# ameli/gaussian-process-param-estimation

Hardware: AMD Instinct MI355X
Metric: log-likelihood evals/sec (N=16384 dense Matern-3/2) (higher is better)
Workload: dtype f64

## Files before the change

gaussian-process-param-estimation_amd/csrc/gpmi_api.hip:

```cpp

#include <hip/hip_runtime.h>

#include <algorithm>
#include <cmath>
#include <cstdarg>
#include <cstdio>
#include <cstdlib>
#include <cstring>
#include <array>
#include <map>
#include <vector>

#include "gpmi_internal.h"
#include "gpmi_host.h"
#include "gpmi_band.h"
#include "gpmi_dense_plan.h"
#include "gpmi_predict_plan.h"
#include "../../include/gpmi.h"

using namespace gpmi;

namespace {

thread_local char g_err[512] = "";

int set_err(int code, const char* fmt, ...) {
  va_list ap;
  va_start(ap, fmt);
  vsnprintf(g_err, sizeof(g_err), fmt, ap);
  va_end(ap);
  return code;
}

constexpr int TS = GPMI_TS;
constexpr int RLD = GPMI_RHS_LD;
constexpr int OUT_LD = 1 + RLD * RLD;

}

struct gpmi_op {
  int device = 0;
  int64_t n = 0, n_pad = 0;
  int nt = 0;
  int max_batch = 1;
  int outer = 16;
  int panel_mode = DENSE_REC;
  hipStream_t stream = nullptr;
  hipStream_t stream3 = nullptr;
  int groups = 0;
  hipEvent_t ev_g = nullptr;
  hipEvent_t ev_fork = nullptr, ev_join = nullptr;
  bool dry = false;
  std::vector<std::pair<int, int>> shapes;
  double* K = nullptr;
  double* A = nullptr;
  double* R = nullptr;
  double* X = nullptr;
  double* U = nullptr;
  double* Linv = nullptr;
  double* logdiag = nullptr;
  double* gram = nullptr;
  double* out = nullptr;
  double* etas = nullptr;
  double* rhs_src = nullptr;
  double* scratch = nullptr;
  double* scratch2 = nullptr;
  double* tracebuf = nullptr;
  double* W = nullptr;
  double* tpart = nullptr;
  double* Td = nullptr;
  int* info = nullptr;
  uint32_t* order = nullptr;
  int order_nt = -1, order_outer = -1, group = 8;
  std::map<std::pair<int, int>, int64_t> order_off;
  int nrhs = 0;
  bool has_K = false;
  bool cache_valid = false;
  double cached_eta = 0.0;
  uint64_t factor_gen = 0;
  uint64_t tinv_gen = ~0ull;
  int tinv_have = 0;
  double tinv[2] = {0.0, 0.0};
  double* PY = nullptr;
  double* PT = nullptr;
  double* Ppart = nullptr;
  double* Pout = nullptr;
  double* Pgram = nullptr;
  int pred_wide = 0;
  int64_t pred_t_rows = 0;
  double* Pcov = nullptr;
  double* Pcpart = nullptr;
  int64_t pred_cov_rows = 0;
  size_t pred_cpart = 0;
  int ncu = 0;
  hipEvent_t cov_ev[2] = {nullptr, nullptr};
  double last_cov_ms = 0.0, last_cov_flops = 0.0;
  int last_cov_split = 0;
  uint64_t rhs_gen = 0;
  uint64_t ry_gen = ~0ull;
  uint64_t ry_rhs = ~0ull;
  uint64_t py_gen = ~0ull, py_rhs = ~0ull;
  std::vector<hipEvent_t> pred_ev;
  double last_pred_ms = 0.0, last_pred_trail_ms = 0.0, last_pred_trail_flops = 0.0;
  bool timing = false;
  std::vector<hipEvent_t> ev;
  hipEvent_t ev_begin = nullptr, ev_end = nullptr;
  double last_syrk_ms = 0.0, last_syrk_flops = 0.0, last_total_ms = 0.0;
  int last_syrk_launches = 0;
  std::vector<std::pair<int, double>> syrk_log;
  std::vector<std::array<int, 3>> syrk_shape;
  double last_syrk_busy_ms = 0.0;
  bool trace = false;
  std::vector<hipEvent_t> colpanel_ev;
  size_t colpanel_ev_used = 0;

  BatchPtrs ptrs() const {
    BatchPtrs p;
    p.A = A;
    p.sA = n_pad * n_pad;
    p.R = R;
    p.sR = n_pad * RLD;
    p.U = U;
    p.sU = (int64_t)TS * RLD;
    p.Linv = Linv;
    p.sL = (int64_t)nt * TS * TS;
    p.logdiag = logdiag;
    p.sLD = nt;
    p.gram = gram;
    p.sG = (int64_t)nt * 256;
    p.info = info;
    return p;
  }
};

namespace {

void grouped_order(int w, int t, int G, std::vector<uint32_t>* out) {
  for (int r0 = 0; r0 < t; r0 += G) {
    const int r1 = std::min(t, r0 + G);
    const int jmax = std::min(r1 - 1, w - 1);
    for (int j = 0; j <= jmax; ++j)
      for (int i = std::max(r0, j); i < r1; ++i) out->push_back(((uint32_t)i << 16) | j);
  }
}

int launch_syrk(gpmi_op* op, hipStream_t st, int b0, int nb, int tc0, int w, int t, int p0,
                int kdim, bool from_k = false) {
  const int tri = w * (w + 1) / 2;
  const int tiles = tri + (t - w) * w;
  if (tiles <= 0 || nb <= 0) return 0;
  if (op->dry) {
    op->shapes.push_back({w, t});
    return 0;
  }
  int evi = -1;
  if (op->timing) {
    evi = (int)op->syrk_log.size() * 2;
    if ((int)op->ev.size() < evi + 2) {
      for (int k = 0; k < 64; ++k) {
        hipEvent_t e;
        HIP_TRY(hipEventCreateWithFlags(&e, timing_event_flags()));
        op->ev.push_back(e);
      }
    }
    HIP_TRY(hipEventRecord(op->ev[evi], st));
  }
  const uint32_t* order = nullptr;
  if (op->order && w > 1) {
    auto it = op->order_off.find({w, t});
    if (it != op->order_off.end()) order = op->order + it->second;
  }
  hipLaunchKernelGGL(syrk_kernel, dim3(tiles, nb), dim3(256), 0, st,
                     op->A + (int64_t)b0 * op->n_pad * op->n_pad, (int64_t)op->n_pad,
                     op->n_pad * op->n_pad, tc0, w, t, p0, kdim, order,
                     from_k ? op->K : nullptr, op->etas + b0, (int64_t)op->n);
  LAUNCH_CHECK("syrk_kernel");
  if (op->timing) {
    HIP_TRY(hipEventRecord(op->ev[evi + 1], st));
    const double offd = (double)(tiles - std::min(tiles, w)) * TS * TS;
    const double diag = (double)std::min(tiles, w) * TS * (TS + 1) / 2.0;
    const double fl = 2.0 * (offd + diag) * kdim * nb;
    op->syrk_log.push_back({evi, fl});
    op->syrk_shape.push_back({w, t, kdim});
  }
  return 0;
}

int factor_panel(gpmi_op* op, const BatchPtrs& P, int nb, hipStream_t st,
                 const DenseLaunch& L) {
  if (op->dry) return 0;
  const int64_t lda = op->n_pad;
  if (L.kind == DENSE_DIAG) {
    hipLaunchKernelGGL(diag_block_kernel, dim3(nb), dim3(256), 0, st, P, lda, L.col, op->nt);
    LAUNCH_CHECK("diag_block_kernel");
  } else if (L.kind == DENSE_PANEL) {
    hipLaunchKernelGGL(panel_kernel, dim3(L.r1 - L.r0, nb), dim3(256), 0, st, P, lda, L.col);
    LAUNCH_CHECK("panel_kernel");
  } else {
    const bool ev = op->timing && op->trace;
    size_t evi = op->colpanel_ev_used;
    if (ev) {
      while (op->colpanel_ev.size() < evi + 2) {
        hipEvent_t e;
        HIP_TRY(hipEventCreateWithFlags(&e, timing_event_flags()));
        op->colpanel_ev.push_back(e);
      }
      HIP_TRY(hipEventRecord(op->colpanel_ev[evi], st));
    }
    hipLaunchKernelGGL(colpanel_kernel, dim3(L.r1 - L.r0, nb), dim3(256), 0, st, P, lda, L.col,
                       L.p0 / TS, L.next_diag ? 1 : 0);
    LAUNCH_CHECK("colpanel_kernel");
    if (ev) {
      HIP_TRY(hipEventRecord(op->colpanel_ev[evi + 1], st));
      op->colpanel_ev_used = evi + 2;
    }
  }
  return 0;
}


int schedule(gpmi_op* op, const BatchPtrs& P, int b0, int nb, hipStream_t main = nullptr) {
  hipStream_t A = main ? main : op->stream;
  for (const DenseLaunch& L : dense_plan(op->nt, op->outer, op->panel_mode)) {
    const int rc = L.kind == DENSE_SYRK
                       ? launch_syrk(op, A, b0, nb, L.col, L.w, L.r1 - L.r0, L.p0, L.kdim,
                                     L.from_k)
                       : factor_panel(op, P, nb, A, L);
    if (rc) return rc;
  }
  return 0;
}

int ensure_order(gpmi_op* op) {
  if (op->group <= 0) return 0;
  if (op->order && op->order_nt == op->nt && op->order_outer == op->outer &&
      true)
    return 0;
  if (op->order) HIP_TRY(hipFree(op->order));
  op->order = nullptr;
  op->order_off.clear();
  op->dry = true;
  op->shapes.clear();
  BatchPtrs P = op->ptrs();
  int rc = schedule(op, P, 0, 1);
  op->dry = false;
  if (rc) return rc;
  std::vector<uint32_t> h;
  for (auto& wt : op->shapes) {
    if (wt.first < 2 || op->order_off.count(wt)) continue;
    op->order_off[wt] = (int64_t)h.size();
    grouped_order(wt.first, wt.second, op->group, &h);
  }
  if (h.empty()) h.push_back(0);
  HIP_TRY(hipMalloc(&op->order, sizeof(uint32_t) * h.size()));
  HIP_TRY(hipMemcpy(op->order, h.data(), sizeof(uint32_t) * h.size(), hipMemcpyHostToDevice));
// ... 225 lines not shown
  int rc = matern_params(nu, &P);
  if (rc) return rc;
  DeviceGuard g(device);
  double *dx = nullptr, *dv = nullptr;
  HIP_TRY(hipMalloc(&dx, sizeof(double) * m));
  HIP_TRY(hipMalloc(&dv, sizeof(double) * m));
  HIP_TRY(hipMemcpy(dx, x, sizeof(double) * m, hipMemcpyHostToDevice));
  hipLaunchKernelGGL(matern_eval_kernel, dim3((unsigned)((m + 255) / 256)), dim3(256), 0, 0, dx,
                     m, P, dv);
  LAUNCH_CHECK("matern_eval_kernel");
  HIP_TRY(hipMemcpy(out, dv, sizeof(double) * m, hipMemcpyDeviceToHost));
  HIP_TRY(hipFree(dx));
  HIP_TRY(hipFree(dv));
  return 0;
}

static int assemble(int device, hipStream_t s, const double* points, int64_t n, int d,
                    const double* scale, double nu, double* Kdev, int64_t ldk,
                    int64_t n_pad) {
  if (d < 1 || d > GPMI_MAX_DIM)
    return set_err(-1003, "dimension %d outside [1, %d]", d, GPMI_MAX_DIM);
  MaternParams P;
  int rc = matern_params(nu, &P);
  if (rc) return rc;
  DeviceGuard g(device);
  double *dp = nullptr, *ds = nullptr;
  HIP_TRY(hipMalloc(&dp, sizeof(double) * std::max<int64_t>(1, n * d)));
  HIP_TRY(hipMalloc(&ds, sizeof(double) * d));
  HIP_TRY(hipMemcpyAsync(dp, points, sizeof(double) * n * d, hipMemcpyHostToDevice, s));
  HIP_TRY(hipMemcpyAsync(ds, scale, sizeof(double) * d, hipMemcpyHostToDevice, s));
  const int64_t T = (n_pad + 63) / 64;
  hipEvent_t e0 = nullptr, e1 = nullptr;
  HIP_TRY(hipEventCreate(&e0));
  HIP_TRY(hipEventCreate(&e1));
  HIP_TRY(hipEventRecord(e0, s));
  launch_matern_dense(dim3((unsigned)(T * (T + 1) / 2)), s, dp, n, d, ds, P, Kdev, ldk, n_pad);
  LAUNCH_CHECK("matern_dense_kernel");
  HIP_TRY(hipEventRecord(e1, s));
  HIP_TRY(hipStreamSynchronize(s));
  float ms = 0.f;
  HIP_TRY(hipEventElapsedTime(&ms, e0, e1));
  g_assembly_ms = ms;
  HIP_TRY(hipEventDestroy(e0));
  HIP_TRY(hipEventDestroy(e1));
  HIP_TRY(hipFree(dp));
  HIP_TRY(hipFree(ds));
  return 0;
}

int gpmi_matern_dense(int device, const double* points, int64_t n, int d,
                      const double* scale, double nu, double* K_out, int64_t ldk) {
  if (n <= 0) return 0;
  DeviceGuard g(device);
  double* dK = nullptr;
  HIP_TRY(hipMalloc(&dK, sizeof(double) * n * n));
  int rc = assemble(device, nullptr, points, n, d, scale, nu, dK, n, n);
  if (rc) {
    (void)hipFree(dK);
    return rc;
  }
  HIP_TRY(hipMemcpy2D(K_out, sizeof(double) * ldk, dK, sizeof(double) * n, sizeof(double) * n,
                      n, hipMemcpyDeviceToHost));
  HIP_TRY(hipFree(dK));
  return 0;
}

int gpmi_op_create(int device, int64_t n, int max_batch, gpmi_op** out) {
  if (!out) return set_err(-1004, "null output handle");
  if (n <= 0) return set_err(-1005, "matrix size must be positive");
  if (max_batch < 1) max_batch = 1;
  DeviceGuard g(device);
  gpmi_op* op = new gpmi_op();
  op->device = device;
  op->n = n;
  op->n_pad = (n + TS - 1) / TS * TS;
  op->nt = (int)(op->n_pad / TS);
  op->max_batch = max_batch;
  if (const char* g = std::getenv("GPMI_GROUPS")) op->groups = std::atoi(g);
  if (const char* m = std::getenv("GPMI_PANEL")) {
    if (!std::strcmp(m, "col")) op->panel_mode = DENSE_COL;
    else if (std::strcmp(m, "rec") && *m) {
      delete op;
      return set_err(-1011, "GPMI_PANEL must be rec or col (got %s)", m);
    }
  }
  op->trace = std::getenv("GPMI_SYRK_TRACE") != nullptr;
  const int64_t np = op->n_pad;
  auto fail = [&](hipError_t e, const char* what) {
    gpmi_op_destroy(op);
    return set_err(-(int)e, "allocation of %s failed: %s", what, hipGetErrorString(e));
  };
  hipError_t e;
  if ((e = hipStreamCreateWithFlags(&op->stream, hipStreamNonBlocking)) != hipSuccess)
    return fail(e, "stream");
  if ((e = hipEventCreateWithFlags(&op->ev_fork, sync_event_flags())) != hipSuccess)
    return fail(e, "event");
  if ((e = hipEventCreateWithFlags(&op->ev_join, sync_event_flags())) != hipSuccess)
    return fail(e, "event");
#define ALLOC(ptr, count)                                                           \
  if ((e = hipMalloc(&op->ptr, sizeof(*op->ptr) * (size_t)(count))) != hipSuccess)  \
    return fail(e, #ptr);
  ALLOC(K, np * np);
  ALLOC(A, (size_t)max_batch * np * np);
  ALLOC(R, (size_t)max_batch * np * RLD);
  ALLOC(X, (size_t)max_batch * np * RLD);
  ALLOC(U, (size_t)max_batch * TS * RLD);
  ALLOC(Linv, (size_t)max_batch * op->nt * TS * TS);
  ALLOC(logdiag, (size_t)max_batch * op->nt);
  ALLOC(gram, (size_t)max_batch * op->nt * 256);
  ALLOC(out, (size_t)max_batch * OUT_LD);
  ALLOC(etas, max_batch);
  ALLOC(rhs_src, np * RLD);
  ALLOC(scratch, np * RLD);
  ALLOC(scratch2, np * RLD);
  ALLOC(tracebuf, np * 2);
  ALLOC(info, max_batch);
#undef ALLOC
  if ((e = hipMemsetAsync(op->rhs_src, 0, sizeof(double) * np * RLD, op->stream)) != hipSuccess)
    return fail(e, "rhs memset");
  if ((e = hipStreamSynchronize(op->stream)) != hipSuccess) return fail(e, "sync");
  *out = op;
  return 0;
}

int gpmi_op_destroy(gpmi_op* op) {
  if (!op) return 0;
  DeviceGuard g(op->device);
  if (op->stream) (void)hipStreamSynchronize(op->stream);
  if (op->stream3) (void)hipStreamSynchronize(op->stream3);
  double* bufs[] = {op->K, op->A, op->R, op->X, op->U, op->Linv, op->logdiag, op->gram,
                    op->out, op->etas, op->rhs_src, op->scratch, op->scratch2, op->tracebuf,
                    op->W, op->tpart, op->Td, op->PY, op->PT, op->Ppart, op->Pout, op->Pgram,
                    op->Pcov, op->Pcpart};
  for (double* p : bufs)
    if (p) (void)hipFree(p);
  if (op->info) (void)hipFree(op->info);
  if (op->order) (void)hipFree(op->order);
  for (auto e : op->ev) (void)hipEventDestroy(e);
  for (auto e : op->colpanel_ev) (void)hipEventDestroy(e);
  for (auto e : op->pred_ev) (void)hipEventDestroy(e);
  for (auto e : op->cov_ev)
    if (e) (void)hipEventDestroy(e);
  if (op->ev_begin) (void)hipEventDestroy(op->ev_begin);
  if (op->ev_end) (void)hipEventDestroy(op->ev_end);
  if (op->ev_fork) (void)hipEventDestroy(op->ev_fork);
  if (op->ev_join) (void)hipEventDestroy(op->ev_join);
  if (op->stream3) (void)hipStreamDestroy(op->stream3);
  if (op->ev_g) (void)hipEventDestroy(op->ev_g);
  if (op->stream) (void)hipStreamDestroy(op->stream);
  delete op;
  return 0;
}

int gpmi_op_size(const gpmi_op* op, int64_t* n, int64_t* n_pad) {
  if (!op) return set_err(-1006, "null handle");
  if (n) *n = op->n;
  if (n_pad) *n_pad = op->n_pad;
  return 0;
}

int gpmi_op_load_matrix(gpmi_op* op, const double* K_host, int64_t ldk) {
  if (!op) return set_err(-1006, "null handle");
  DeviceGuard g(op->device);
  const int64_t np = op->n_pad, n = op->n;
  std::vector<double> pad_rows;
  HIP_TRY(hipMemsetAsync(op->K, 0, sizeof(double) * np * np, op->stream));
// ... 671 lines not shown
```

gaussian-process-param-estimation_amd/csrc/gpmi_chol.hip:

```cpp

#include <hip/hip_runtime.h>
#include <math.h>
#include <stdint.h>

#include "gpmi_internal.h"

#include "gpmi_device.h"

namespace gpmi {

__global__ __launch_bounds__(256) void shift_copy_kernel(
    const double* __restrict__ K, int64_t ldk, double* __restrict__ A, int64_t lda,
    int64_t sA, const double* __restrict__ etas, int nb, int64_t n, int wc) {
  int I, J;
  tri_decode(blockIdx.x, wc, &I, &J);
  const int t = threadIdx.x;
  for (int e = t; e < TS * TS / 2; e += 256) {
    const int r = e >> 6, c = (e & 63) * 2;
    const int64_t gi = (int64_t)I * TS + r, gj = (int64_t)J * TS + c;
    const d2 v = *reinterpret_cast<const d2*>(K + gi * ldk + gj);
    for (int b = 0; b < nb; ++b) {
      d2 o = v;
      if (gi < n) {
        if (gi == gj) o[0] += etas[b];
// ... 48 lines not shown
#pragma unroll
  for (int it = 0; it < 4; ++it) v[it] = *reinterpret_cast<const d2*>(U + 2 * (it * 256 + t));
#pragma unroll
  for (int it = 0; it < 4; ++it) *reinterpret_cast<d2*>(&sU[2 * (it * 256 + t)]) = v[it];
}

__device__ __forceinline__ void wg_global_barrier() {
  __builtin_amdgcn_fence(__ATOMIC_RELEASE, "workgroup");
  __syncthreads();
  __builtin_amdgcn_fence(__ATOMIC_ACQUIRE, "workgroup");
}

__global__ __launch_bounds__(256, 2) void panel_kernel(BatchPtrs P, int64_t lda, int kb) {
  __shared__ double smem[4 * STAGE + TS * RLD];
  double* sU = smem + 4 * STAGE;
  const int b = blockIdx.y;
  const int I = kb + 1 + blockIdx.x;
  double* A = P.A + b * P.sA;
  if (!GPMI_PROBE_PANEL_NO_RHS) stage_u(P.U + b * P.sU, sU);
  panel_step(A + (int64_t)I * TS * lda + (int64_t)kb * TS, lda,
             P.Linv + b * P.sL + (int64_t)kb * TS * TS,
             P.R + b * P.sR + (int64_t)I * TS * RLD, smem, smem + 2 * STAGE, sU);
}

__device__ __forceinline__ void load_c(const double* C, int64_t lda, d4 (&acc)[4][4]) {
  const int tid = threadIdx.x, lane = tid & 63, wv = tid >> 6;
  const int wr = wv >> 1, wc = wv & 1, fr = lane & 15, fk = lane >> 4;
#pragma unroll
  for (int a = 0; a < 4; ++a)
#pragma unroll
    for (int c = 0; c < 4; ++c)
#pragma unroll
      for (int r = 0; r < 4; ++r)
        acc[a][c][r] = C[(int64_t)(wr * 64 + a * 16 + fk + 4 * r) * lda + wc * 64 + c * 16 + fr];
}
__device__ __forceinline__ void store_c(double* C, int64_t lda, const d4 (&acc)[4][4]) {
  const int tid = threadIdx.x, lane = tid & 63, wv = tid >> 6;
  const int wr = wv >> 1, wc = wv & 1, fr = lane & 15, fk = lane >> 4;
#pragma unroll
  for (int a = 0; a < 4; ++a)
#pragma unroll
    for (int c = 0; c < 4; ++c)
#pragma unroll
      for (int r = 0; r < 4; ++r)
        C[(int64_t)(wr * 64 + a * 16 + fk + 4 * r) * lda + wc * 64 + c * 16 + fr] = acc[a][c][r];
}

__global__ __launch_bounds__(256, 2) void colpanel_kernel(BatchPtrs P, int64_t lda, int kb,
                                                          int c0, int next_diag) {
  __shared__ double smem[4 * STAGE + TS * RLD];
  double* sA = smem;
  double* sB = smem + 2 * STAGE;
  double* sU = smem + 4 * STAGE;
  const int b = blockIdx.y;
  const int I = kb + 1 + blockIdx.x;
  const int kdim = (kb - c0) * TS;
  double* A = P.A + b * P.sA;
  stage_u(P.U + b * P.sU, sU);
  double* rowI = A + (int64_t)I * TS * lda;
  double* Aik = rowI + (int64_t)kb * TS;
  d4 dummy[2];
  if (kdim > 0) {
    d4 acc[4][4];
    load_c(Aik, lda, acc);
    tile_mma<false, true>(rowI + (int64_t)c0 * TS, lda,
                          A + (int64_t)kb * TS * lda + (int64_t)c0 * TS, lda, kdim, sA, sB, acc,
                          nullptr, dummy);
    store_c(Aik, lda, acc);
    wg_global_barrier();
  }
  panel_step(Aik, lda, P.Linv + b * P.sL + (int64_t)kb * TS * TS,
             P.R + b * P.sR + (int64_t)I * TS * RLD, sA, sB, sU);
  if (next_diag && blockIdx.x == 0) {
    wg_global_barrier();
    double* D = rowI + (int64_t)I * TS;
    d4 acc[4][4];
    load_c(D, lda, acc);
    tile_mma<false, true>(rowI + (int64_t)c0 * TS, lda, rowI + (int64_t)c0 * TS, lda,
                          kdim + TS, sA, sB, acc, nullptr, dummy);
    store_c(D, lda, acc);
  }
}

__global__ __launch_bounds__(256, 2) void syrk_kernel(double* A, int64_t lda, int64_t sA,
                                                      int tc0, int w, int t, int p0,
                                                      int kdim, const uint32_t* order,
                                                      const double* __restrict__ Ksrc,
                                                      const double* __restrict__ etas,
                                                      int64_t n) {
  __shared__ double smem[4 * STAGE];
  const int tid = threadIdx.x, lane = tid & 63, wv = tid >> 6;
  const int wr = wv >> 1, wc = wv & 1, fr = lane & 15, fk = lane >> 4;
  const int q = xcd_remap(blockIdx.x, gridDim.x);
  int i, j;
  if (order) {
    const uint32_t o = order[q];
    i = (int)(o >> 16);
    j = (int)(o & 0xffffu);
  } else {
    tri_decode(q, w, &i, &j);
  }
  (void)t;
  const int I = tc0 + i, J = tc0 + j;
  double* Ab = A + blockIdx.y * sA;
  const double* P1 = Ab + (int64_t)I * TS * lda + p0;
  const double* P2 = Ab + (int64_t)J * TS * lda + p0;
  double* C = Ab + (int64_t)I * TS * lda + (int64_t)J * TS;
  const double* Cin = Ksrc ? Ksrc + (int64_t)I * TS * lda + (int64_t)J * TS : C;
  d4 acc[4][4];
  load_c(Cin, lda, acc);
  if (Ksrc && I == J && wr == wc) {
    const double eta = etas[blockIdx.y];
#pragma unroll
    for (int a = 0; a < 4; ++a)
#pragma unroll
      for (int r = 0; r < 4; ++r)
        if (fk + 4 * r == fr && (int64_t)I * TS + wr * 64 + a * 16 + fr < n) acc[a][a][r] += eta;
  }
  d4 dummy[2];
  tile_mma<false, true>(P1, lda, P2, lda, kdim, smem, smem + 2 * STAGE, acc, nullptr, dummy);
  store_c(C, lda, acc);
}

__global__ __launch_bounds__(256) void finalize_kernel(BatchPtrs P, int nt, double* out,
                                                       int out_ld) {
  const int b = blockIdx.x, t = threadIdx.x;
  double g = 0.0;
  for (int k = 0; k < nt; ++k) g += P.gram[b * P.sG + (int64_t)k * 256 + t];
  out[b * out_ld + 1 + t] = g;
  if (t == 0) {
    double s = 0.0;
    for (int k = 0; k < nt; ++k) s += P.logdiag[b * P.sLD + k];
    out[b * out_ld] = s;
  }
}

__global__ __launch_bounds__(256) void bwd_step_kernel(BatchPtrs P, int64_t lda, int kb,
                                                       double* X, int64_t sX) {
  __shared__ double Ys[TS * RLD];
  __shared__ double Xs[TS * RLD];
  const int t = threadIdx.x, b = blockIdx.y, jblk = blockIdx.x;
  const int row = t & 127, half = t >> 7;
  double* R = P.R + b * P.sR;
  const double* A = P.A + b * P.sA;
  const double* Li = P.Linv + b * P.sL + (int64_t)kb * TS * TS;
  for (int e = t; e < TS * RLD; e += 256) Ys[e] = R[(int64_t)kb * TS * RLD + e];
  __syncthreads();
  {
    double xv[8];
#pragma unroll
    for (int q = 0; q < 8; ++q) xv[q] = 0.0;
    for (int r = row; r < TS; ++r) {
      const double l = Li[r * TS + row];
#pragma unroll
      for (int q = 0; q < 8; ++q) xv[q] += l * Ys[r * RLD + half * 8 + q];
    }
#pragma unroll
    for (int q = 0; q < 8; ++q) Xs[row * RLD + half * 8 + q] = xv[q];
  }
  __syncthreads();
  if (jblk == 0) {
    double* Xb = X + b * sX + (int64_t)kb * TS * RLD;
    for (int e = t; e < TS * RLD; e += 256) Xb[e] = Xs[e];
  }
  if (kb == 0) return;
  const double* Lkj = A + (int64_t)kb * TS * lda + (int64_t)jblk * TS;
  const int c = row;
  double yv[8];
#pragma unroll
  for (int q = 0; q < 8; ++q) yv[q] = 0.0;
  for (int r = 0; r < TS; ++r) {
    const double l = Lkj[(int64_t)r * lda + c];
#pragma unroll
    for (int q = 0; q < 8; ++q) yv[q] += l * Xs[r * RLD + half * 8 + q];
  }
  double* Yj = R + (int64_t)jblk * TS * RLD;
#pragma unroll
  for (int q = 0; q < 8; ++q) Yj[c * RLD + half * 8 + q] -= yv[q];
}

__global__ __launch_bounds__(256) void gemv_sym_kernel(const double* __restrict__ K,
                                                       int64_t ldk, int64_t n,
                                                       const double* __restrict__ x,
                                                       int64_t ldx, int ncol,
                                                       double* __restrict__ y, double eta,
                                                       int exponent) {
  (void)eta;
  (void)exponent;
  const int lane = threadIdx.x & 63;
  const int64_t row = (int64_t)blockIdx.x * 4 + (threadIdx.x >> 6);
  if (row >= n) return;
  for (int c = 0; c < ncol; ++c) {
    double s = 0.0;
    for (int64_t j = lane; j < n; j += 64) s += K[row * ldk + j] * x[j * ldx + c];
#pragma unroll
    for (int off = 32; off > 0; off >>= 1) s += __shfl_xor(s, off);
    if (lane == 0) y[row * ldx + c] = s;
  }
}

__global__ __launch_bounds__(256) void trace_kernel(const double* __restrict__ K, int64_t ldk,
                                                    int64_t n, double* __restrict__ out) {
  __shared__ double s0[256], s1[256];
  const int t = threadIdx.x;
  const int64_t row = blockIdx.x;
// ... 72 lines not shown
```

gaussian-process-param-estimation_amd/csrc/gpmi_device.h:

```cpp
#pragma once

#include <hip/hip_runtime.h>
#include <stdint.h>

#include "gpmi_internal.h"

namespace gpmi {

typedef double d4 __attribute__((ext_vector_type(4)));
typedef double d2 __attribute__((ext_vector_type(2)));

constexpr int TS = GPMI_TS;
constexpr int BK = 16;
constexpr int STAGE = TS * BK;

__device__ __forceinline__ int slab_off(int row, int k) {
  return row * BK + 2 * ((k >> 1) ^ ((row >> 1) & 7)) + (k & 1);
}
constexpr int RLD = GPMI_RHS_LD;

__device__ __forceinline__ void st_sc1(double* p, double v) {
  __hip_atomic_store(reinterpret_cast<unsigned long long*>(p),
                     (unsigned long long)__double_as_longlong(v), __ATOMIC_RELAXED,
                     __HIP_MEMORY_SCOPE_AGENT);
}
__device__ __forceinline__ double ld_sc1(const double* p) {
  return __longlong_as_double((long long)__hip_atomic_load(
      reinterpret_cast<const unsigned long long*>(p), __ATOMIC_RELAXED,
      __HIP_MEMORY_SCOPE_AGENT));
}

__device__ __forceinline__ d4 mfma64(double a, double b, d4 c) {
  return __builtin_amdgcn_mfma_f64_16x16x4f64(a, b, c, 0, 0, 0);
}

__device__ __forceinline__ d4 mfma64_neg(double a, double b, d4 c) {
  return __builtin_amdgcn_mfma_f64_16x16x4f64(a, b, c, 0, 0, 1);
}


__device__ __forceinline__ void gload_slab(const double* __restrict__ base, int64_t ld,
                                           int p, d2 (&r)[4]) {
  const int t = threadIdx.x;
#pragma unroll
  for (int i = 0; i < 4; ++i) {
    const int idx = i * 256 + t;
    const int row = idx >> 3, c2 = idx & 7;
    r[i] = *reinterpret_cast<const d2*>(base + (int64_t)row * ld + p + 2 * c2);
  }
}

__device__ __forceinline__ void sstore_slab(double* s, const d2 (&r)[4]) {
  const int t = threadIdx.x;
#pragma unroll
  for (int i = 0; i < 4; ++i) {
    const int idx = i * 256 + t;
    const int row = idx >> 3, c2 = idx & 7;
    *reinterpret_cast<d2*>(s + row * BK + 2 * (c2 ^ ((row >> 1) & 7))) = r[i];
  }
}


template <bool WITH_RHS, bool NEG = false>
__device__ __forceinline__ void tile_mma(const double* __restrict__ P1, int64_t ld1,
                                         const double* __restrict__ P2, int64_t ld2,
                                         int kdim, double* sA, double* sB,
                                         d4 (&acc)[4][4], const double* sU,
                                         d4 (&racc)[2]) {
  const int t = threadIdx.x, lane = t & 63, w = t >> 6;
  const int wr = w >> 1, wc = w & 1;
  const int fr = lane & 15, fk = lane >> 4;
  d2 ra[4], rb[4];
  gload_slab(P1, ld1, 0, ra);
  gload_slab(P2, ld2, 0, rb);
  sstore_slab(sA, ra);
  sstore_slab(sB, rb);
  __syncthreads();
  __builtin_amdgcn_s_waitcnt(0x0F70);
  const int nsteps = kdim / BK;
  for (int s = 0; s < nsteps; ++s) {
    const int cur = s & 1;
    const double* cA = sA + cur * STAGE;
    const double* cB = sB + cur * STAGE;
    if (s + 1 < nsteps) {
      gload_slab(P1, ld1, (s + 1) * BK, ra);
      gload_slab(P2, ld2, (s + 1) * BK, rb);
    }
#pragma unroll
    for (int kk = 0; kk < BK / 4; ++kk) {
      double a[4], b[4];
#pragma unroll
      for (int i = 0; i < 4; ++i) a[i] = cA[slab_off(wr * 64 + i * 16 + fr, kk * 4 + fk)];
#pragma unroll
      for (int j = 0; j < 4; ++j) b[j] = cB[slab_off(wc * 64 + j * 16 + fr, kk * 4 + fk)];
#pragma unroll
      for (int i = 0; i < 4; ++i)
#pragma unroll
        for (int j = 0; j < 4; ++j)
          acc[i][j] = NEG ? mfma64_neg(a[i], b[j], acc[i][j]) : mfma64(a[i], b[j], acc[i][j]);
      if (WITH_RHS) {
        const double u = sU[(s * BK + kk * 4 + fk) * RLD + fr];
        const double a0 = wc ? a[2] : a[0];
        const double a1 = wc ? a[3] : a[1];
        racc[0] = mfma64(a0, u, racc[0]);
        racc[1] = mfma64(a1, u, racc[1]);
      }
    }
    if (s + 1 < nsteps) {
      sstore_slab(sA + (cur ^ 1) * STAGE, ra);
      sstore_slab(sB + (cur ^ 1) * STAGE, rb);
    }
    __syncthreads();
  }
}

__device__ __forceinline__ int trsm_cb(int wc, int j) { return 2 * j + ((j ^ wc) & 1); }

template <bool WITH_RHS>
__device__ __forceinline__ void tile_trsm(const double* P1, int64_t ld1, const double* Linv,
                                          double* sA, double* sB, d4 (&acc)[4][4],
                                          const double* sU, d4 (&racc)[2]) {
  const int t = threadIdx.x, lane = t & 63;
  const int w = __builtin_amdgcn_readfirstlane(t >> 6);
  const int wr = w >> 1, wc = w & 1;
  const int fr = lane & 15, fk = lane >> 4;
  d2 ra[4], rb[4];
  gload_slab(P1, ld1, 0, ra);
  gload_slab(Linv, TS, 0, rb);
  sstore_slab(sA, ra);
  sstore_slab(sB, rb);
  __syncthreads();
  constexpr int nsteps = TS / BK;
#pragma unroll
  for (int s = 0; s < nsteps; ++s) {
    const int cur = s & 1;
    const double* cA = sA + cur * STAGE;
    const double* cB = sB + cur * STAGE;
    if (s + 1 < nsteps) {
      gload_slab(P1, ld1, (s + 1) * BK, ra);
      gload_slab(Linv, TS, (s + 1) * BK, rb);
    }
#pragma unroll
    for (int kk = 0; kk < BK / 4; ++kk) {
      double a[4];
#pragma unroll
      for (int i = 0; i < 4; ++i) a[i] = cA[slab_off(wr * 64 + i * 16 + fr, kk * 4 + fk)];
#pragma unroll
      for (int j = 0; j < 4; ++j) {
        if (s <= 2 * j || (s == 2 * j + 1 && ((j ^ wc) & 1))) {
          const double bj = cB[slab_off(trsm_cb(wc, j) * 16 + fr, kk * 4 + fk)];
#pragma unroll
// ... 43 lines not shown
```

gaussian-process-param-estimation_amd/csrc/gpmi_internal.h:

```cpp
#pragma once

#include <hip/hip_runtime.h>
#include <stdint.h>
#include <stdlib.h>

#include "gpmi_ms_sched.h"

#define GPMI_MAX_DIM 8
#define GPMI_TS 128
#define GPMI_RHS_LD 16

struct gpmi_sp;

namespace gpmi {

inline unsigned sync_event_flags() {
  static const unsigned f = [] {
    const char* e = getenv("GPMI_EV_SYSFENCE");
    return (unsigned)hipEventDisableTiming |
           ((e && e[0] == '1') ? 0u : (unsigned)hipEventDisableSystemFence);
  }();
  return f;
}
inline unsigned timing_event_flags() {
  return sync_event_flags() & ~(unsigned)hipEventDisableTiming;
}

enum MaternMode { MATERN_HALF = 0, MATERN_3HALF = 1, MATERN_5HALF = 2,
                  MATERN_GENERAL = 3, MATERN_GAUSS = 4 };

struct MaternParams {
  int mode;
  double nu;
  double sqrt2nu;
  double mu;
  double lp0, lp1;
};

void launch_matern_dense(dim3 grid, hipStream_t s, const double* points, int64_t n, int d,
                         const double* scale, const MaternParams& P, double* K, int64_t ldk,
                         int64_t n_pad);

struct BatchPtrs {
  double* A;        int64_t sA;
  double* R;        int64_t sR;
  double* U;        int64_t sU;
  double* Linv;     int64_t sL;
  double* logdiag;  int64_t sLD;
  double* gram;     int64_t sG;
  int* info;
};

__global__ void shift_copy_kernel(const double* K, int64_t ldk, double* A, int64_t lda,
                                  int64_t sA, const double* etas, int nb, int64_t n,
                                  int wc);
__global__ void diag_block_kernel(BatchPtrs P, int64_t lda, int kb, int nt);
__global__ void panel_kernel(BatchPtrs P, int64_t lda, int kb);
__global__ void colpanel_kernel(BatchPtrs P, int64_t lda, int kb, int c0, int next_diag);
__global__ void syrk_kernel(double* A, int64_t lda, int64_t sA, int tc0, int w, int t,
                            int p0, int kdim, const uint32_t* order, const double* Ksrc,
                            const double* etas, int64_t n);
__global__ void finalize_kernel(BatchPtrs P, int nt, double* out, int out_ld);
__global__ void bwd_step_kernel(BatchPtrs P, int64_t lda, int kb, double* X, int64_t sX);
__global__ void fwd_step_kernel(BatchPtrs P, int64_t lda, int kb);
__global__ void gemv_sym_kernel(const double* K, int64_t ldk, int64_t n,
                                const double* x, int64_t ldx, int ncol, double* y,
                                double eta, int exponent);
__global__ void trace_kernel(const double* K, int64_t ldk, int64_t n, double* out);
__global__ void trinv_diag_kernel(const double* Linv, double* W, int64_t ldw, int k,
                                  double* partial);
__global__ void trinv_update_kernel(const double* L, int64_t lda, double* W, int64_t ldw, int i0,
                                    int nj, int kb, int ke);
__global__ void gram_panel_kernel(double* W, int64_t ldw, double* Td, int p0, int kdim,
                                  int imax);
__global__ void gram_sumsq_kernel(const double* W, int64_t ldw, const double* Td,
                                  double* partial);
__global__ void matern_eval_kernel(const double* x, int64_t m, MaternParams P, double* out);

void launch_matern_cross(hipStream_t s, const double* points, int64_t n, const double* test,
                         int64_t ns, int d, const double* scale, const MaternParams& P,
                         double* C, int64_t ldc, int64_t rows, int64_t cols);

__global__ void pred_update_kernel(const double* L, int64_t lda, double* T, int64_t ldt, int i0,
                                   int ni, int nct, int kb, int ke);
__global__ void pred_diag_kernel(const double* L, int64_t lda, const double* Linv,
                                 const double* Y, double* T, int64_t ldt, int k, int kb,
                                 double* part, int64_t ns_ld);
__global__ void pred_reduce_kernel(const double* part, int nt, int64_t cnt, double* out);
__global__ void pred_gram_kernel(const double* Y, double* gpart);
__global__ void pred_cov_partial_kernel(const double* T, int64_t ldt, int nct, int nt, int S,
                                        double* part);
__global__ void pred_cov_reduce_kernel(const double* part, int S, int nct, double* C,
                                       int64_t ldc);

#ifndef GPMI_LZ_JC
#define GPMI_LZ_JC 16
#endif
constexpr int LZ_JC = GPMI_LZ_JC;

struct MsScal {
  double* rr;
  double* a;
  double* a_prev;
  double* beta;
  int* active;
};
struct MsShift {
  double* bn2;
  double* z;
  double* z_prev;
  double* bp;
  double* g;
  int* flags;
  int* it_stop;
};
constexpr int MS_UB = 512;
constexpr int MS_DOT_BLK = 256;

constexpr int MS_CJOBS = 12;
struct MsCompactJob {
  const double* src;
  double* dst;
  int64_t rows;
  int L;
  int pad;
};
struct MsCompactArgs {
  MsCompactJob job[MS_CJOBS];
  int njob, s, a, nd, s0, pad;
  int map[MS_MAXS];
  int drop[MS_MAXS];
  int drop_orig[MS_MAXS];
  const double* g;
  double* gfin;
  int64_t SN;
  const int* act_src;
  int* act;
};

int sp_scatter_dense(const ::gpmi_sp* sp, int device, double* K, int64_t ldk,
                     hipStream_t st);
// ... 3 lines not shown
```

gaussian-process-param-estimation_amd/csrc/gpmi_predict.hip:

```cpp

#include <hip/hip_runtime.h>
#include <stdint.h>

#include "gpmi_internal.h"
#include "gpmi_device.h"
#include "gpmi_predict_plan.h"

namespace gpmi {

namespace {

__device__ __forceinline__ void load_c(const double* C, int64_t ldc, d4 (&acc)[4][4]) {
  const int tid = threadIdx.x, lane = tid & 63, wv = tid >> 6;
  const int wr = wv >> 1, wc = wv & 1, fr = lane & 15, fk = lane >> 4;
#pragma unroll
  for (int a = 0; a < 4; ++a)
#pragma unroll
    for (int c = 0; c < 4; ++c)
#pragma unroll
      for (int r = 0; r < 4; ++r)
        acc[a][c][r] = C[(int64_t)(wr * 64 + a * 16 + fk + 4 * r) * ldc + wc * 64 + c * 16 + fr];
}

__device__ __forceinline__ void store_c(double* C, int64_t ldc, const d4 (&acc)[4][4]) {
  const int tid = threadIdx.x, lane = tid & 63, wv = tid >> 6;
  const int wr = wv >> 1, wc = wv & 1, fr = lane & 15, fk = lane >> 4;
#pragma unroll
  for (int a = 0; a < 4; ++a)
#pragma unroll
    for (int c = 0; c < 4; ++c)
#pragma unroll
      for (int r = 0; r < 4; ++r)
        C[(int64_t)(wr * 64 + a * 16 + fk + 4 * r) * ldc + wc * 64 + c * 16 + fr] = acc[a][c][r];
}

__device__ __forceinline__ void store_transposed(double* T, int64_t ldt, const d4 (&acc)[4][4]) {
  const int t = threadIdx.x, lane = t & 63, w = t >> 6;
  const int wr = w >> 1, wc = w & 1, fr = lane & 15, fk = lane >> 4;
#pragma unroll
  for (int a = 0; a < 4; ++a)
#pragma unroll
    for (int c = 0; c < 4; ++c)
#pragma unroll
      for (int r = 0; r < 4; ++r)
        T[(int64_t)(wc * 64 + c * 16 + fr) * ldt + wr * 64 + a * 16 + fk + 4 * r] = acc[a][c][r];
}

__device__ __forceinline__ void wg_global_barrier() {
  __builtin_amdgcn_fence(__ATOMIC_RELEASE, "workgroup");
  __syncthreads();
  __builtin_amdgcn_fence(__ATOMIC_ACQUIRE, "workgroup");
}

}

__global__ __launch_bounds__(256, 2) void pred_update_kernel(const double* __restrict__ L,
                                                             int64_t lda, double* T,
                                                             int64_t ldt, int i0, int ni,
                                                             int nct, int kb, int ke) {
  __shared__ double smem[4 * STAGE];
  const int q = xcd_remap(blockIdx.x, gridDim.x);
  int i, j;
  predict_tile(q, ni, nct, &i, &j);
  i += i0;
  double* rowJ = T + (int64_t)j * TS * ldt;
  double* C = rowJ + (int64_t)i * TS;
  d4 acc[4][4];
  load_c(C, ldt, acc);
  d4 dummy[2];
  tile_mma<false, true>(rowJ + (int64_t)kb * TS, ldt, L + (int64_t)i * TS * lda + (int64_t)kb * TS,
                        lda, (ke - kb) * TS, smem, smem + 2 * STAGE, acc, nullptr, dummy);
  store_c(C, ldt, acc);
}

__global__ __launch_bounds__(256, 2) void pred_diag_kernel(const double* __restrict__ L,
                                                           int64_t lda,
                                                           const double* __restrict__ Linv,
                                                           const double* __restrict__ Y,
                                                           double* T, int64_t ldt, int k, int kb,
                                                           double* __restrict__ part,
                                                           int64_t ns_ld) {
  __shared__ double smem[4 * STAGE + TS * RLD];
  double* sA = smem;
  double* sB = smem + 2 * STAGE;
  double* sY = smem + 4 * STAGE;
  const int j = blockIdx.x;
  const int t = threadIdx.x, lane = t & 63, w = t >> 6;
  const int wr = w >> 1, wc = w & 1, fr = lane & 15, fk = lane >> 4;
  double* rowJ = T + (int64_t)j * TS * ldt;
  double* Tjk = rowJ + (int64_t)k * TS;
  {
    const double* Yk = Y + (int64_t)k * TS * RLD;
    d2 v[4];
#pragma unroll
    for (int it = 0; it < 4; ++it) v[it] = *reinterpret_cast<const d2*>(Yk + 2 * (it * 256 + t));
#pragma unroll
    for (int it = 0; it < 4; ++it) *reinterpret_cast<d2*>(&sY[2 * (it * 256 + t)]) = v[it];
  }
  d4 acc[4][4];
  d4 dummy[2];
  if (k > kb) {
    load_c(Tjk, ldt, acc);
    tile_mma<false, true>(rowJ + (int64_t)kb * TS, ldt,
                          L + (int64_t)k * TS * lda + (int64_t)kb * TS, lda, (k - kb) * TS, sA, sB,
                          acc, nullptr, dummy);
    store_c(Tjk, ldt, acc);
    wg_global_barrier();
  }
#pragma unroll
  for (int a = 0; a < 4; ++a)
#pragma unroll
    for (int c = 0; c < 4; ++c) acc[a][c] = d4{0.0, 0.0, 0.0, 0.0};
  tile_mma<false>(Linv + (int64_t)k * TS * TS, TS, Tjk, ldt, TS, sA, sB, acc, nullptr, dummy);
  store_transposed(Tjk, ldt, acc);
  d4 ep[4];
  double qs[4];
#pragma unroll
  for (int c = 0; c < 4; ++c) {
    ep[c] = d4{0.0, 0.0, 0.0, 0.0};
    qs[c] = 0.0;
  }
#pragma unroll
  for (int a = 0; a < 4; ++a)
#pragma unroll
    for (int r = 0; r < 4; ++r) {
      const double y = sY[(wr * 64 + a * 16 + 4 * r + fk) * RLD + fr];
#pragma unroll
      for (int c = 0; c < 4; ++c) {
        ep[c] = mfma64(y, acc[a][c][r], ep[c]);
        qs[c] = fma(acc[a][c][r], acc[a][c][r], qs[c]);
      }
    }
#pragma unroll
  for (int c = 0; c < 4; ++c) {
    qs[c] += __shfl_xor(qs[c], 16);
    qs[c] += __shfl_xor(qs[c], 32);
  }
  double* red = smem;
  if (wr == 1) {
#pragma unroll
    for (int c = 0; c < 4; ++c) {
      double* o = red + (wc * 4 + c) * PRED_LD * 16;
#pragma unroll
      for (int r = 0; r < 4; ++r) o[(fk + 4 * r) * 16 + fr] = ep[c][r];
      if (fk == 0) o[16 * 16 + fr] = qs[c];
    }
  }
  __syncthreads();
  if (wr == 0) {
#pragma unroll
    for (int c = 0; c < 4; ++c) {
      const double* o = red + (wc * 4 + c) * PRED_LD * 16;
      double* out = part + ((int64_t)k * ns_ld + (int64_t)j * TS + wc * 64 + c * 16 + fr) * PRED_LD;
#pragma unroll
// ... 87 lines not shown
```

Measured before the change: 45.16.

## Add early-issue software-pipelined k-loop with buffer loads and pinned MFMA schedule

Adds a new tile_mma variant that issues global loads two stages ahead using raw buffer loads with scalar offsets. It uses sched_group_barrier hints to interleave the MFMA, LDS-read and global-load instructions, and prefetches LDS fragments for the next k-step. The syrk and predict-update kernels use it by default, with tile indices made wave-uniform via readfirstlane. The goal is to hide global and LDS latency behind MFMA work in the dominant trailing update, at the cost of more registers and a fragile hand-pinned schedule. It also assumes kdim is a multiple of 2*BK.

```diff
diff --git a/gaussian-process-param-estimation_amd/csrc/gpmi_api.hip b/gaussian-process-param-estimation_amd/csrc/gpmi_api.hip
--- a/gaussian-process-param-estimation_amd/csrc/gpmi_api.hip
+++ b/gaussian-process-param-estimation_amd/csrc/gpmi_api.hip
@@ -45,6 +45,7 @@
   int max_batch = 1;
   int outer = 16;
   int panel_mode = DENSE_REC;
+  int kloop = KLOOP_EARLY;
   hipStream_t stream = nullptr;
   hipStream_t stream3 = nullptr;
   int groups = 0;
@@ -170,7 +171,8 @@
     auto it = op->order_off.find({w, t});
     if (it != op->order_off.end()) order = op->order + it->second;
   }
-  hipLaunchKernelGGL(syrk_kernel, dim3(tiles, nb), dim3(256), 0, st,
+  hipLaunchKernelGGL(op->kloop == KLOOP_LATE ? syrk_kernel<KLOOP_LATE> : syrk_kernel<KLOOP_EARLY>,
+                     dim3(tiles, nb), dim3(256), 0, st,
                      op->A + (int64_t)b0 * op->n_pad * op->n_pad, (int64_t)op->n_pad,
                      op->n_pad * op->n_pad, tc0, w, t, p0, kdim, order,
                      from_k ? op->K : nullptr, op->etas + b0, (int64_t)op->n);
@@ -562,6 +564,13 @@
     else if (std::strcmp(m, "rec") && *m) {
       delete op;
       return set_err(-1011, "GPMI_PANEL must be rec or col (got %s)", m);
+    }
+  }
+  if (const char* m = std::getenv("GPMI_KLOOP")) {
+    if (!std::strcmp(m, "late")) op->kloop = KLOOP_LATE;
+    else if (std::strcmp(m, "early") && *m) {
+      delete op;
+      return set_err(-1009, "GPMI_KLOOP must be early or late (got %s)", m);
     }
   }
   op->trace = std::getenv("GPMI_SYRK_TRACE") != nullptr;
diff --git a/gaussian-process-param-estimation_amd/csrc/gpmi_chol.hip b/gaussian-process-param-estimation_amd/csrc/gpmi_chol.hip
--- a/gaussian-process-param-estimation_amd/csrc/gpmi_chol.hip
+++ b/gaussian-process-param-estimation_amd/csrc/gpmi_chol.hip
@@ -154,6 +154,7 @@
   }
 }
 
+template <int KL>
 __global__ __launch_bounds__(256, 2) void syrk_kernel(double* A, int64_t lda, int64_t sA,
                                                       int tc0, int w, int t, int p0,
                                                       int kdim, const uint32_t* order,
@@ -173,6 +174,10 @@
     tri_decode(q, w, &i, &j);
   }
   (void)t;
+  if (KL == KLOOP_EARLY) {
+    i = __builtin_amdgcn_readfirstlane(i);
+    j = __builtin_amdgcn_readfirstlane(j);
+  }
   const int I = tc0 + i, J = tc0 + j;
   double* Ab = A + blockIdx.y * sA;
   const double* P1 = Ab + (int64_t)I * TS * lda + p0;
@@ -190,9 +195,15 @@
         if (fk + 4 * r == fr && (int64_t)I * TS + wr * 64 + a * 16 + fr < n) acc[a][a][r] += eta;
   }
   d4 dummy[2];
-  tile_mma<false, true>(P1, lda, P2, lda, kdim, smem, smem + 2 * STAGE, acc, nullptr, dummy);
+  tile_mma<false, true, KL>(P1, lda, P2, lda, kdim, smem, smem + 2 * STAGE, acc, nullptr, dummy);
   store_c(C, lda, acc);
 }
+template __global__ void syrk_kernel<KLOOP_LATE>(double*, int64_t, int64_t, int, int, int, int,
+                                                 int, const uint32_t*, const double*,
+                                                 const double*, int64_t);
+template __global__ void syrk_kernel<KLOOP_EARLY>(double*, int64_t, int64_t, int, int, int, int,
+                                                  int, const uint32_t*, const double*,
+                                                  const double*, int64_t);
 
 __global__ __launch_bounds__(256) void finalize_kernel(BatchPtrs P, int nt, double* out,
                                                        int out_ld) {
diff --git a/gaussian-process-param-estimation_amd/csrc/gpmi_device.h b/gaussian-process-param-estimation_amd/csrc/gpmi_device.h
--- a/gaussian-process-param-estimation_amd/csrc/gpmi_device.h
+++ b/gaussian-process-param-estimation_amd/csrc/gpmi_device.h
@@ -61,12 +61,151 @@
 }
 
 
-template <bool WITH_RHS, bool NEG = false>
+__device__ __forceinline__ __amdgpu_buffer_rsrc_t slab_rsrc(const double* base) {
+  return __builtin_amdgcn_make_buffer_rsrc(const_cast<double*>(base), 0, 0xffffffff, 0x00020000);
+}
+__device__ __forceinline__ uint32_t slab_voff(int64_t ld) {
+  const int t = threadIdx.x;
+  return (uint32_t)(((t >> 3) * ld + 2 * (t & 7)) * 8);
+}
+__device__ __forceinline__ void gload_slab_u(__amdgpu_buffer_rsrc_t rs, int64_t ld, int p,
+                                             uint32_t voff, d2 (&r)[4]) {
+#pragma unroll
+  for (int i = 0; i < 4; ++i) {
+    const uint32_t soff = (uint32_t)(((int64_t)(i * 32) * ld + p) * 8);
+    r[i] = __builtin_bit_cast(d2, __builtin_amdgcn_raw_buffer_load_b128(rs, voff, soff, 0));
+  }
+}
+
+template <int MASK, int N, int PER>
+__device__ __forceinline__ void pin_behind_mfma() {
+#pragma unroll
+  for (int q = 0; q < N; ++q) {
+    __builtin_amdgcn_sched_group_barrier(0x8, 1, 0);
+    __builtin_amdgcn_sched_group_barrier(MASK, PER, 0);
+  }
+}
+template <int LEAD>
+__device__ __forceinline__ void pin_kstep() {
+  if (LEAD > 0) __builtin_amdgcn_sched_group_barrier(0x8, LEAD, 0);
+  pin_behind_mfma<0x100, 4, 1>();
+  __builtin_amdgcn_sched_group_barrier(0x8, 12 - LEAD, 0);
+}
+
+template <bool WITH_RHS, bool NEG, int CUR>
+__device__ __forceinline__ void tile_mma_early_stage(
+    __amdgpu_buffer_rsrc_t R1, int64_t ld1, __amdgpu_buffer_rsrc_t R2, int64_t ld2,
+    uint32_t vo1, uint32_t vo2, int s, bool has2, double* sA, double* sB, d4 (&acc)[4][4],
+    const double* sU, d4 (&racc)[2], d2 (&ra)[4], d2 (&rb)[4], double (&a)[4],
+    double (&b)[4]) {
+  const int t = threadIdx.x, lane = t & 63, w = t >> 6;
+  const int wr = w >> 1, wc = w & 1;
+  const int fr = lane & 15, fk = lane >> 4;
+  const double* cA = sA + CUR * STAGE;
+  const double* cB = sB + CUR * STAGE;
+  double* nA = sA + (CUR ^ 1) * STAGE;
+  double* nB = sB + (CUR ^ 1) * STAGE;
+  sstore_slab(nA, ra);
+  sstore_slab(nB, rb);
+#pragma unroll
+  for (int kk = 0; kk < BK / 4; ++kk) {
+    double an[4], bn[4];
+#pragma unroll
+    for (int i = 0; i < 4; ++i) {
+      if (kk == 0 && i == 1) {
+        pin_behind_mfma<0x200, 4, 2>();
+        if (has2) {
+          gload_slab_u(R1, ld1, (s + 2) * BK, vo1, ra);
+          gload_slab_u(R2, ld2, (s + 2) * BK, vo2, rb);
+        }
+      }
+      if ((kk == 0 && i == 1) || (kk > 0 && i == 0)) {
+        const double* fA = kk + 1 < BK / 4 ? cA : nA;
+        const double* fB = kk + 1 < BK / 4 ? cB : nB;
+        const int kn = ((kk + 1) * 4) % BK + fk;
+#pragma unroll
+        for (int ii = 0; ii < 4; ++ii) an[ii] = fA[slab_off(wr * 64 + ii * 16 + fr, kn)];
+#pragma unroll
+        for (int j = 0; j < 4; ++j) bn[j] = fB[slab_off(wc * 64 + j * 16 + fr, kn)];
+      }
+#pragma unroll
+      for (int j = 0; j < 4; ++j)
+        acc[i][j] = NEG ? mfma64_neg(a[i], b[j], acc[i][j]) : mfma64(a[i], b[j], acc[i][j]);
+    }
+    if (WITH_RHS) {
+      const double u = sU[(s * BK + kk * 4 + fk) * RLD + fr];
+      const double a0 = wc ? a[2] : a[0];
+      const double a1 = wc ? a[3] : a[1];
+      racc[0] = mfma64(a0, u, racc[0]);
+      racc[1] = mfma64(a1, u, racc[1]);
+    }
+#pragma unroll
+    for (int i = 0; i < 4; ++i) {
+      a[i] = an[i];
+      b[i] = bn[i];
+    }
+    if (kk == 1) {
+      __builtin_amdgcn_sched_group_barrier(0x8, 4, 0);
+      pin_behind_mfma<0x100, 4, 1>();
+      __builtin_amdgcn_sched_group_barrier(0x8, 4, 0);
+      pin_kstep<0>();
+      __builtin_amdgcn_sched_barrier(0);
+      __syncthreads();
+      __builtin_amdgcn_sched_barrier(0);
+    }
+  }
+  pin_kstep<8>();
+  pin_kstep<0>();
+  __builtin_amdgcn_sched_barrier(0);
+  __syncthreads();
+  __builtin_amdgcn_sched_barrier(0);
+}
+
+template <bool WITH_RHS, bool NEG>
+__device__ __forceinline__ void tile_mma_early(const double* __restrict__ P1, int64_t ld1,
+                                               const double* __restrict__ P2, int64_t ld2,
+                                               int kdim, double* sA, double* sB,
+                                               d4 (&acc)[4][4], const double* sU,
+                                               d4 (&racc)[2]) {
+  const int t = threadIdx.x, lane = t & 63, w = t >> 6;
+  const int wr = w >> 1, wc = w & 1;
+  const int fr = lane & 15, fk = lane >> 4;
+  const int nsteps = kdim / BK;
+  const uint32_t vo1 = slab_voff(ld1), vo2 = slab_voff(ld2);
+  const __amdgpu_buffer_rsrc_t R1 = slab_rsrc(P1), R2 = slab_rsrc(P2);
+  d2 ra[4], rb[4];
+  gload_slab_u(R1, ld1, 0, vo1, ra);
+  gload_slab_u(R2, ld2, 0, vo2, rb);
+  sstore_slab(sA, ra);
+  sstore_slab(sB, rb);
+  __builtin_amdgcn_s_waitcnt(0x0F70);
+  gload_slab_u(R1, ld1, BK, vo1, ra);
+  gload_slab_u(R2, ld2, BK, vo2, rb);
+  __syncthreads();
+  double a[4], b[4];
+#pragma unroll
+  for (int i = 0; i < 4; ++i) a[i] = sA[slab_off(wr * 64 + i * 16 + fr, fk)];
+#pragma unroll
+  for (int j = 0; j < 4; ++j) b[j] = sB[slab_off(wc * 64 + j * 16 + fr, fk)];
+  __builtin_amdgcn_sched_barrier(0);
+  for (int s = 0; s < nsteps; s += 2) {
+    tile_mma_early_stage<WITH_RHS, NEG, 0>(R1, ld1, R2, ld2, vo1, vo2, s, s + 2 < nsteps, sA, sB,
+                                           acc, sU, racc, ra, rb, a, b);
+    tile_mma_early_stage<WITH_RHS, NEG, 1>(R1, ld1, R2, ld2, vo1, vo2, s + 1, s + 3 < nsteps, sA,
+                                           sB, acc, sU, racc, ra, rb, a, b);
+  }
+}
+
+template <bool WITH_RHS, bool NEG = false, int KL = KLOOP_LATE>
 __device__ __forceinline__ void tile_mma(const double* __restrict__ P1, int64_t ld1,
                                          const double* __restrict__ P2, int64_t ld2,
                                          int kdim, double* sA, double* sB,
                                          d4 (&acc)[4][4], const double* sU,
                                          d4 (&racc)[2]) {
+  if constexpr (KL == KLOOP_EARLY) {
+    tile_mma_early<WITH_RHS, NEG>(P1, ld1, P2, ld2, kdim, sA, sB, acc, sU, racc);
+    return;
+  }
   const int t = threadIdx.x, lane = t & 63, w = t >> 6;
   const int wr = w >> 1, wc = w & 1;
   const int fr = lane & 15, fk = lane >> 4;
diff --git a/gaussian-process-param-estimation_amd/csrc/gpmi_internal.h b/gaussian-process-param-estimation_amd/csrc/gpmi_internal.h
--- a/gaussian-process-param-estimation_amd/csrc/gpmi_internal.h
+++ b/gaussian-process-param-estimation_amd/csrc/gpmi_internal.h
@@ -57,6 +57,8 @@
 __global__ void diag_block_kernel(BatchPtrs P, int64_t lda, int kb, int nt);
 __global__ void panel_kernel(BatchPtrs P, int64_t lda, int kb);
 __global__ void colpanel_kernel(BatchPtrs P, int64_t lda, int kb, int c0, int next_diag);
+enum { KLOOP_LATE = 0, KLOOP_EARLY = 1 };
+template <int KL>
 __global__ void syrk_kernel(double* A, int64_t lda, int64_t sA, int tc0, int w, int t,
                             int p0, int kdim, const uint32_t* order, const double* Ksrc,
                             const double* etas, int64_t n);
diff --git a/gaussian-process-param-estimation_amd/csrc/gpmi_predict.hip b/gaussian-process-param-estimation_amd/csrc/gpmi_predict.hip
--- a/gaussian-process-param-estimation_amd/csrc/gpmi_predict.hip
+++ b/gaussian-process-param-estimation_amd/csrc/gpmi_predict.hip
@@ -62,14 +62,16 @@
   const int q = xcd_remap(blockIdx.x, gridDim.x);
   int i, j;
   predict_tile(q, ni, nct, &i, &j);
-  i += i0;
+  i = __builtin_amdgcn_readfirstlane(i) + i0;
+  j = __builtin_amdgcn_readfirstlane(j);
   double* rowJ = T + (int64_t)j * TS * ldt;
   double* C = rowJ + (int64_t)i * TS;
   d4 acc[4][4];
   load_c(C, ldt, acc);
   d4 dummy[2];
-  tile_mma<false, true>(rowJ + (int64_t)kb * TS, ldt, L + (int64_t)i * TS * lda + (int64_t)kb * TS,
-                        lda, (ke - kb) * TS, smem, smem + 2 * STAGE, acc, nullptr, dummy);
+  tile_mma<false, true, KLOOP_EARLY>(rowJ + (int64_t)kb * TS, ldt,
+                                     L + (int64_t)i * TS * lda + (int64_t)kb * TS, lda,
+                                     (ke - kb) * TS, smem, smem + 2 * STAGE, acc, nullptr, dummy);
   store_c(C, ldt, acc);
 }
 
```

Result: faster. 48.36 (median of 6 runs) (+7.1%).
